# QuEraComputing/tsim

Hardware: AMD Instinct MI355X
Metric: detector shots/sec, 35-qubit distillation circuit, 1/2/4/8 MI355X (higher is better)
Workload: dtype int32

## Files before the change

tsim_amd/csrc/tsim_kernel_hw.hip.h:

```cpp
#pragma once
#include "tsim_kernels.hip.h"
#include "tsim_kernel4.hip.h"

namespace tsimk {

#define TSIMK_HW_MAX_CTX 8
struct HwMulti {
  int n_ctx, waves_per_list, max_lists;
  int comp_par;
  int par_words;
  uint32_t slot_cap;
  uint32_t hw_blocks;
  int comp4_off;
  uint32_t *feedback;
  SampleArgs ctx[TSIMK_HW_MAX_CTX];
};

__device__ __forceinline__ int hw_sum_i32(int v) {
#pragma unroll
  for (int o = 32; o > 0; o >>= 1) v += __shfl_xor(v, o, 64);
  return v;
}
__device__ __forceinline__ uint32_t hw_or_u32(uint32_t v) {
#pragma unroll
  for (int o = 32; o > 0; o >>= 1) v |= (uint32_t)__shfl_xor((int)v, o, 64);
  return v;
}

__device__ __forceinline__ uint32_t hw_bits(const uint32_t *par, uint32_t pos, uint32_t n) {
  const uint32_t w = pos >> 5, sh = pos & 31u;
  const uint32_t lo = par[w], hi = par[w + 1u];
  const uint32_t v = __builtin_amdgcn_alignbit(hi, lo, sh);
  return n >= 32u ? v : (v & ((1u << n) - 1u));
}

struct HwLevelOut {
  float re, im, re0, im0;
};

template <int W>
__device__ __forceinline__ void hw_phase1(const uint32_t *gimg, cptr lvl, const uint32_t (&x)[W], bool hasA, uint32_t flipA, bool hasB,
                                          uint32_t flipB, uint32_t *par, uint32_t pw, uint32_t wv, uint32_t nwv) {
  const uint32_t lane = threadIdx.x & 63u;
  const uint32_t n_rows = lvl[L_HWN];
  const uint32_t *rows = gimg + lvl[L_HWROWS];
  const uint32_t steps = (n_rows + 63u) >> 6;
  const uint32_t aw = flipA >> 5, as = flipA & 31u, bw = flipB >> 5, bs = flipB & 31u;
#pragma unroll 8
  for (uint32_t st = wv; st < steps; st += nwv) {
    const uint32_t r = st * 64u + lane;
    uint32_t pb = 0u, fa = 0u, fb = 0u;
    if (r < n_rows) {
      const uint32_t *q = rows + (size_t)r * (W + 1);
      uint32_t rw[W + 1];
#pragma unroll
      for (int w = 0; w <= W; ++w) rw[w] = q[w];
      uint32_t t = rw[W] & x[W - 1];
#pragma unroll
      for (int w = W - 2; w >= 0; --w) t = and_xor(rw[1 + w], x[w], t);
      pb = ((uint32_t)__builtin_popcount(t) + rw[0]) & 1u;
      uint32_t wa = rw[1], wb = rw[1];
#pragma unroll
      for (int w = 1; w < W; ++w) {
        wa = (aw == (uint32_t)w) ? rw[1 + w] : wa;
        wb = (bw == (uint32_t)w) ? rw[1 + w] : wb;
      }
      fa = (wa >> as) & 1u;
      fb = (wb >> bs) & 1u;
    }
    const unsigned long long m0 = __builtin_amdgcn_ballot_w64(pb != 0u);
    unsigned long long m1 = 0ull, m2 = 0ull, m3 = 0ull;
    if (hasA) m1 = __builtin_amdgcn_ballot_w64((pb ^ fa) != 0u);
    if (hasB) m2 = __builtin_amdgcn_ballot_w64((pb ^ fb) != 0u);
    if (hasA && hasB) m3 = __builtin_amdgcn_ballot_w64((pb ^ fa ^ fb) != 0u);
    if (lane == 0u) {
      par[2u * st] = (uint32_t)m0;
      par[2u * st + 1u] = (uint32_t)(m0 >> 32);
      if (hasA) { par[pw + 2u * st] = (uint32_t)m1; par[pw + 2u * st + 1u] = (uint32_t)(m1 >> 32); }
      if (hasB) { par[2u * pw + 2u * st] = (uint32_t)m2; par[2u * pw + 2u * st + 1u] = (uint32_t)(m2 >> 32); }
      if (hasA && hasB) { par[3u * pw + 2u * st] = (uint32_t)m3; par[3u * pw + 2u * st + 1u] = (uint32_t)(m3 >> 32); }
    }
  }
  if (lane == 0u && wv == (steps % nwv)) {
    par[2u * steps] = 0u;
    par[pw + 2u * steps] = 0u;
    par[2u * pw + 2u * steps] = 0u;
    par[3u * pw + 2u * steps] = 0u;
  }
}

typedef uint32_t hw_u32x4 __attribute__((ext_vector_type(4)));
struct HwRec {
  hw_u32x4 r0, r1, r2, r3;
};
__device__ __forceinline__ HwRec hw_load_rec(const uint32_t *gimg, cptr lvl, uint32_t g) {
  HwRec R;
  R.r0 = R.r1 = R.r2 = R.r3 = hw_u32x4{0u, 0u, 0u, 0u};
  if (g < lvl[L_G]) {
    const hw_u32x4 *q4 = reinterpret_cast<const hw_u32x4 *>(gimg + lvl[L_GRAPHS] + (size_t)g * G_WORDS);
    R.r0 = q4[0]; R.r1 = q4[1]; R.r2 = q4[2]; R.r3 = q4[3];
  }
  return R;
}

template <int W, bool DUAL>
__device__ __forceinline__ HwLevelOut hw_phase2(const uint32_t *gimg, cptr img, cptr lvl, const uint32_t *pa, const uint32_t *pa0, const HwRec &first) {
  const uint32_t G = lvl[L_G];
  const bool approx = (lvl[L_FLAGS] & TSIMK_LFLAG_APPROX) != 0;
  const bool fixed = (lvl[L_FLAGS] & TSIMK_LFLAG_FIXED) != 0;
  const uint32_t graphs = lvl[L_GRAPHS];
  const uint32_t lane = threadIdx.x & 63u;
  hw_u32x4 rec0 = first.r0, rec1 = first.r1, rec2 = first.r2, rec3 = first.r3;
  auto load_rec = [&](uint32_t g) {
    const hw_u32x4 *q4 = reinterpret_cast<const hw_u32x4 *>(gimg + graphs + (size_t)g * G_WORDS);
    rec0 = q4[0]; rec1 = q4[1]; rec2 = q4[2]; rec3 = q4[3];
  };
  LevelSum S, S0;
  for (uint32_t g0 = 0; g0 < G; g0 += 64u) {
    const uint32_t g = g0 + lane;
    const bool mine = g < G;
    int a = 0, b = 0, c = 0, d = 0, p = 0, a0 = 0, b0 = 0, c0 = 0, d0 = 0, p0 = 0;
    float tr = 0.0f, ti = 0.0f, tr0 = 0.0f, ti0 = 0.0f;
    if (mine && g0 > 0u) load_rec(g);
    if (mine) {
      const uint32_t n01 = rec0.x, n3h = rec0.y, flags = rec0.z, nD = rec0.w;
      const uint32_t start = rec2.x;
      static_assert(GF_N01 == 0 && GF_N3H == 1 && GF_FLAGS == 2 && GF_ND == 3 && GF_TBL == 5 && GF_N1 == 6 && GF_TBL2 == 7 && GF_HWROW == 8 &&
                        GF_APRE == 11 && GF_APIM == 12 && G_WORDS == 16, "record words are taken from the four 16-byte loads by position");
      GraphRec R;
      R.flags = flags; R.nD = nD; R.n1 = rec1.z; R.tbl = rec1.y; R.tbl2 = rec1.w;
      const uint32_t apre = rec2.w, apim = rec3.x;
      auto bits_of = [&](const uint32_t *pq) {
        GraphBits q;
        uint32_t pos = start;
        const uint32_t n0 = n01 & 0xFFFFu, n1 = n01 >> 16, n3 = n3h & 0xFFFFu;
        auto count = [&](uint32_t n) -> uint32_t {
          uint32_t m = (uint32_t)__builtin_popcount(hw_bits(pq, pos, n));
          for (uint32_t t0 = 32u; t0 < n; t0 += 32u) m += (uint32_t)__builtin_popcount(hw_bits(pq, pos + t0, n - t0));
          pos += n;
          return m;
        };
        q.m0 = count(n0);
        q.m1 = count(n1);
        q.m3 = count(n3);
        q.dbits = 0u;
        for (uint32_t t0 = 0; t0 < nD; t0 += 16u) {
          const uint32_t nt = min(16u, nD - t0);
          const uint32_t bits = hw_bits(pq, pos, 2u * nt);
          for (uint32_t t = 0; t < nt; ++t) q.dbits = (q.dbits << 2) | ((bits >> (2u * t)) & 3u);
          pos += 2u * nt;
        }
        q.lam = 0u;
        q.e = 0u;
        if (flags & TSIMK_GFLAG_LAM) { q.lam = hw_bits(pq, pos, 1u); pos += 1u; }
        if (flags & TSIMK_GFLAG_LIN) { q.e = hw_bits(pq, pos, 1u); pos += 1u; }
        const uint32_t nH = n3h >> 16;
        for (uint32_t t0 = 0; t0 < nH; t0 += 16u) {
          const uint32_t nt = min(16u, nH - t0);
          const uint32_t bits = hw_bits(pq, pos, 2u * nt);
          q.e ^= (uint32_t)__builtin_popcount(bits & (bits >> 1) & 0x55555555u);
          pos += 2u * nt;
        }
        return q;
      };
      const GraphBits q1 = bits_of(pa);
      graph_fast_value(gimg, R, fixed, q1, a, b, c, d, p);
      if (approx) level_term_approx(apre, apim, a, b, c, d, p, tr, ti);
      if constexpr (DUAL) {
        const GraphBits q0 = bits_of(pa0);
        graph_fast_value(gimg, R, fixed, q0, a0, b0, c0, d0, p0);
        if (approx) level_term_approx(apre, apim, a0, b0, c0, d0, p0, tr0, ti0);
      }
    }
    if (fixed) {
      S.sa += a; S.sb += b; S.sc += c; S.sd += d;
      if constexpr (DUAL) { S0.sa += a0; S0.sb += b0; S0.sc += c0; S0.sd += d0; }
    } else {
      const uint32_t n = min(64u, G - g0);
      for (uint32_t l = 0; l < n; ++l) {
        if (approx) {
          S.fre = __fadd_rn(S.fre, __uint_as_float((uint32_t)__builtin_amdgcn_readlane((int)__float_as_uint(tr), (int)l)));
          S.fim = __fadd_rn(S.fim, __uint_as_float((uint32_t)__builtin_amdgcn_readlane((int)__float_as_uint(ti), (int)l)));
          if constexpr (DUAL) {
            S0.fre = __fadd_rn(S0.fre, __uint_as_float((uint32_t)__builtin_amdgcn_readlane((int)__float_as_uint(tr0), (int)l)));
            S0.fim = __fadd_rn(S0.fim, __uint_as_float((uint32_t)__builtin_amdgcn_readlane((int)__float_as_uint(ti0), (int)l)));
          }
        } else {
          level_sum_exact(S, __builtin_amdgcn_readlane(a, (int)l), __builtin_amdgcn_readlane(b, (int)l), __builtin_amdgcn_readlane(c, (int)l),
                          __builtin_amdgcn_readlane(d, (int)l), __builtin_amdgcn_readlane(p, (int)l));
          if constexpr (DUAL)
            level_sum_exact(S0, __builtin_amdgcn_readlane(a0, (int)l), __builtin_amdgcn_readlane(b0, (int)l), __builtin_amdgcn_readlane(c0, (int)l),
                            __builtin_amdgcn_readlane(d0, (int)l), __builtin_amdgcn_readlane(p0, (int)l));
        }
      }
    }
  }
  if (fixed) {
    S.sa = hw_sum_i32(S.sa); S.sb = hw_sum_i32(S.sb); S.sc = hw_sum_i32(S.sc); S.sd = hw_sum_i32(S.sd);
    if constexpr (DUAL) { S0.sa = hw_sum_i32(S0.sa); S0.sb = hw_sum_i32(S0.sb); S0.sc = hw_sum_i32(S0.sc); S0.sd = hw_sum_i32(S0.sd); }
  }
  HwLevelOut o;
  o.re = o.im = o.re0 = o.im0 = 0.0f;
  level_finish(S, lvl, approx, fixed, o.re, o.im, nullptr);
  if constexpr (DUAL) level_finish(S0, lvl, approx, fixed, o.re0, o.im0, nullptr);
  return o;
}

template <int W, class FBit>
__device__ __forceinline__ void hw_component(const SampleArgs &A, cptr img, cptr comp, int ci, FBit fbit, unsigned long long shot, bool check,
                                             uint32_t *par, uint32_t pw, uint32_t (&out_w)[4]) {
  const uint32_t lane = threadIdx.x & 63u;
  const uint32_t wv = threadIdx.x >> 6, nwv = blockDim.x >> 6;
  const bool lead = wv == 0u;
  const uint32_t n_out = comp[C_NOUT], F = comp[C_F];
  cptr fsel = img + comp[C_FSEL];
  cptr levels = img + comp[C_LEVELS];
  cptr outpos = img + comp[C_OUTPOS];
  const uint32_t keybase = comp[C_KEYBASE];
  uint32_t *bit_word = par + 8u * pw;
  uint32_t x[W];
#pragma unroll
  for (int w2 = 0; w2 < W; w2 += 2) {
    const uint32_t j = 32u * (uint32_t)w2 + lane;
    const uint32_t raw = fbit(fsel[j < F ? j : 0u]);
    const unsigned long long m = __builtin_amdgcn_ballot_w64(j < F && raw != 0u);
    x[w2] = (uint32_t)m;
    if (w2 + 1 < W) x[w2 + 1] = (uint32_t)(m >> 32);
  }
  uint32_t u_bits = 0u;
  if (lead && n_out > 0u) {
    const uint32_t o = keybase + (lane < n_out ? lane : 0u);
    uint32_t x0 = (uint32_t)(shot >> 32), x1 = (uint32_t)shot;
    threefry2x32(subkey(A, o, 0), subkey(A, o, 1), x0, x1);
    u_bits = __float_as_uint(__uint_as_float(((x0 ^ x1) >> 9) | 0x3F800000u) - 1.0f);
  }
  auto set_bit = [&](uint32_t pos, bool on) {
    const uint32_t wi = pos >> 5, bm = 1u << (pos & 31u);
#pragma unroll
    for (int w = 0; w < W; ++w)
      if ((uint32_t)w == wi) x[w] = on ? (x[w] | bm) : (x[w] & ~bm);
  };
  HwRec cur = lead ? hw_load_rec(A.img, levels, lane) : HwRec{};
  hw_phase1<W>(A.img, levels, x, false, 0u, false, 0u, par, pw, wv, nwv);
  __syncthreads();
  float prev = 0.0f, maxdev = 0.0f;
  if (n_out > 0u) set_bit(F, true);
  if (lead) {
    const HwRec nxt = n_out > 0u ? hw_load_rec(A.img, levels + L_WORDS, lane) : HwRec{};
    const HwLevelOut n0 = hw_phase2<W, false>(A.img, img, levels, par, par, cur);
    prev = cabs32(n0.re, n0.im);
    cur = nxt;
  } else if (n_out > 0u) {
    hw_phase1<W>(A.img, levels + L_WORDS, x, false, 0u, check, F, par + 4u * pw, pw, wv - 1u, nwv - 1u);
  }
  __syncthreads();
  uint32_t prev_bit = 1u;
  for (uint32_t i = 0; i < n_out; ++i) {
    cptr lvl = levels + (i + 1) * L_WORDS;
    const uint32_t bitpos = F + i;
    uint32_t *buf = par + (((i + 1u) & 1u) ? 4u * pw : 0u);
    if (lead) {
      const uint32_t *pa = buf + (prev_bit ? 0u : pw);
      const HwRec nxt = i + 1u < n_out ? hw_load_rec(A.img, lvl + L_WORDS, lane) : HwRec{};
      float p1;
      if (check) {
        const HwLevelOut o = hw_phase2<W, true>(A.img, img, lvl, pa, pa + 2u * pw, cur);
        p1 = cabs32(o.re, o.im);
        const float p0 = cabs32(o.re0, o.im0);
        const float norm = __fdiv_rn(__fadd_rn(p0, p1), prev);
        maxdev = nanmax(maxdev, fabsf(__fsub_rn(norm, 1.0f)));
      } else {
        const HwLevelOut o = hw_phase2<W, false>(A.img, img, lvl, pa, pa, cur);
        p1 = cabs32(o.re, o.im);
      }
      const float u = __uint_as_float((uint32_t)__builtin_amdgcn_readlane((int)u_bits, (int)i));
      const bool bit = u < __fdiv_rn(p1, prev);
      prev = bit ? p1 : __fsub_rn(prev, p1);
      if (lane == 0u) *bit_word = bit ? 1u : 0u;
      cur = nxt;
    } else if (i + 1u < n_out) {
      uint32_t xn[W];
#pragma unroll
      for (int w = 0; w < W; ++w) xn[w] = x[w];
      const uint32_t np = bitpos + 1u, wi = np >> 5, bm = 1u << (np & 31u);
#pragma unroll
      for (int w = 0; w < W; ++w)
        if ((uint32_t)w == wi) xn[w] |= bm;
      hw_phase1<W>(A.img, lvl + L_WORDS, xn, true, bitpos, check, np, par + (((i + 2u) & 1u) ? 4u * pw : 0u), pw, wv - 1u, nwv - 1u);
    }
    __syncthreads();
    const bool bit = *bit_word != 0u;
    prev_bit = bit ? 1u : 0u;
    set_bit(bitpos, bit);
    if (i + 1u < n_out) set_bit(bitpos + 1u, true);
    const uint32_t dst = outpos[i];
    if (lane == 0u) {
#pragma unroll
      for (int w = 0; w < 4; ++w)
        if ((dst >> 5) == (uint32_t)w) out_w[w] |= (bit ? 1u : 0u) << (dst & 31u);
    }
  }
  if (check && A.norm_dev && threadIdx.x == 0u) A.norm_dev[ci] = maxdev;
  __syncthreads();
}


template <int WMAX>
__device__ __forceinline__ void hw_row(const SampleArgs &A, long long row, bool check, uint32_t *par, uint32_t pw, int only_comp) {
  cptr img = (cptr)(uintptr_t)A.img;
  const uint32_t lane = threadIdx.x & 63u;
  const unsigned long long shot = (unsigned long long)(A.shot_offset + row);
  const int WF32 = 2 * A.WF;
  const uint32_t *frow = reinterpret_cast<const uint32_t *>(A.f + row * A.WF);
  const uint32_t fw = (int)lane < WF32 ? frow[lane] : 0u;
  auto fbit = [&](uint32_t src) -> uint32_t {
    const uint32_t wv = (uint32_t)__shfl((int)fw, (int)(src >> 5), 64);
    return (wv >> (src & 31u)) & 1u;
  };
  uint32_t out_w[4] = {0u, 0u, 0u, 0u};
  if (only_comp < 0) {
    cptr dt = img + A.direct_off;
    for (int j0 = 0; j0 < A.n_direct; j0 += 64) {
      const int j = j0 + (int)lane;
      const bool mine = j < A.n_direct;
      const int jc = mine ? j : 0;
      const uint32_t s = dt[2 * jc], dst = mine ? dt[2 * jc + 1] : 0u;
      const uint32_t raw = fbit(s & 0x7FFFFFFFu);
      const uint32_t bit = mine ? (raw ^ (s >> 31)) : 0u;
#pragma unroll
      for (int w = 0; w < 4; ++w)
        if ((dst >> 5) == (uint32_t)w) out_w[w] |= bit << (dst & 31u);
    }
  }
  for (int ci = only_comp < 0 ? 0 : only_comp; ci < (only_comp < 0 ? A.n_comp : only_comp + 1); ++ci) {
    cptr comp = img + A.comp_off + ci * C_WORDS;
    switch (comp[C_W]) {
      case 1:
        hw_component<1>(A, img, comp, ci, fbit, shot, check, par, pw, out_w);
        break;
      case 2:
        if constexpr (WMAX >= 2) {
          hw_component<2>(A, img, comp, ci, fbit, shot, check, par, pw, out_w);
        }
        break;
      case 3:
      case 4:
        if constexpr (WMAX >= 4) {
          if (comp[C_W] == 3u) hw_component<3>(A, img, comp, ci, fbit, shot, check, par, pw, out_w);
          else hw_component<4>(A, img, comp, ci, fbit, shot, check, par, pw, out_w);
        }
        break;
      case 6:
      case 8:
        if constexpr (WMAX >= 8) {
          if (comp[C_W] == 6u) hw_component<6>(A, img, comp, ci, fbit, shot, check, par, pw, out_w);
          else hw_component<8>(A, img, comp, ci, fbit, shot, check, par, pw, out_w);
        }
        break;
      default: __builtin_trap();
    }
  }
#pragma unroll
  for (int w = 0; w < 4; ++w) out_w[w] = hw_or_u32(out_w[w]);
  if (threadIdx.x == 0u && only_comp >= 0) {
    if (A.out) {
      uint32_t *orow = reinterpret_cast<uint32_t *>(A.out + row * A.WO);
#pragma unroll
      for (int w = 0; w < 4; ++w)
        if (w < 2 * A.WO && out_w[w]) atomicOr(orow + w, out_w[w]);
    }
    if (A.out_compact) {
      const unsigned long long at = (unsigned long long)row * (unsigned long long)A.out_rb;
      uint32_t *base = reinterpret_cast<uint32_t *>(A.out_compact + (at & ~3ull));
      const uint32_t sh = 8u * (uint32_t)(at & 3ull);
#pragma unroll
      for (int w = 0; w < 5; ++w) {
        const uint32_t cur = w < 4 ? out_w[w < 4 ? w : 0] : 0u, below = w > 0 ? out_w[w > 0 ? w - 1 : 0] : 0u;
        const uint32_t v = sh ? ((cur << sh) | (below >> (32u - sh))) : cur;
        if (v) atomicOr(base + w, v);
      }
    }
  } else if (threadIdx.x == 0u) {
    if (A.out) {
      uint64_t *orow = A.out + row * A.WO;
      for (int w = 0; w < A.WO; ++w) orow[w] = (uint64_t)out_w[2 * w] | ((uint64_t)out_w[2 * w + 1] << 32);
    }
    if (A.out_compact) {
      uint8_t *dst = A.out_compact + row * A.out_rb;
      for (int k = 0; k < A.out_rb; ++k) dst[k] = (uint8_t)(out_w[k >> 2] >> (8 * (k & 3)));
    }
  }
}

template <int W, int NCH>
__global__ void __launch_bounds__(256) k_sample_hw(HwMulti M) {
  if constexpr (NCH > 0) {
    if (blockIdx.x >= M.hw_blocks) {
      over4_rows<4, NCH>(M.ctx, M.n_ctx, M.comp4_off, M.slot_cap, M.comp_par > 1, blockIdx.x - M.hw_blocks, gridDim.x - M.hw_blocks);
      return;
    }
  }
  __builtin_amdgcn_s_setprio(3);
  const uint32_t cp = (uint32_t)M.comp_par;
  const uint32_t wv = blockIdx.x / cp;
  const int only_comp = cp > 1u ? (int)(blockIdx.x - wv * cp) : -1;
  const uint32_t per_ctx = (uint32_t)(M.max_lists * M.waves_per_list);
  const uint32_t c = wv / per_ctx;
  if (c >= (uint32_t)M.n_ctx) return;
  const uint32_t r = wv - c * per_ctx;
  const SampleArgs &A = M.ctx[c];
  const uint32_t k = r / (uint32_t)M.waves_per_list, j = r - k * (uint32_t)M.waves_per_list;
  const uint32_t lane = threadIdx.x & 63u;
  if (M.feedback && blockIdx.x == 0u && threadIdx.x < 64u) {
    uint32_t cn = (int)lane < A.row_lists ? A.row_count[32u * lane] : 0u, mx = cn;
#pragma unroll
    for (int o = 32; o > 0; o >>= 1) {
      cn += (uint32_t)__shfl_xor((int)cn, o, 64);
      mx = max(mx, (uint32_t)__shfl_xor((int)mx, o, 64));
    }
    if (lane == 0u) {
      M.feedback[0] = cn;
      M.feedback[1] = mx;
      M.feedback[2] = (uint32_t)min(A.B, 0xFFFFFFFFll);
    }
  }
  if ((int)k >= A.row_lists) return;
  uint32_t n = A.row_count[32u * k];
  if (M.slot_cap) n = min(n, M.slot_cap);
  const uint32_t check_row = (A.no_check || !A.check_row) ? 0xFFFFFFFFu : *A.check_row;
  for (uint32_t slot = j; slot < n; slot += (uint32_t)M.waves_per_list) {
    const uint32_t entry = A.row_index[(size_t)k * A.row_list_cap + slot];
    if (only_comp >= 0) {
      if (!((entry >> (28 + only_comp)) & 1u)) continue;
      const uint32_t row = entry & 0x0FFFFFFFu;
      hw_row<W>(A, (long long)row, row == check_row, tsimk_lds, (uint32_t)M.par_words, only_comp);
    } else {
      hw_row<W>(A, (long long)entry, entry == check_row, tsimk_lds, (uint32_t)M.par_words, -1);
    }
  }
}

}
```

tsim_amd/csrc/tsim_sample.hip:

```cpp
#include "tsim_internal.hip.h"

#include <chrono>
#include "tsim_kernel4h.hip.h"
#include "tsim_filter.hip.h"
#include "tsim_lw_pass.hip.h"
#include "tsim_lw_multi.hip.h"
#include "tsim_lw_fast.hip.h"
#include "tsim_kernel4w.hip.h"
#include "tsim_kernel_hw.hip.h"
#include "tsim_direct.hip.h"
#include "tsim_lw_fastm.hip.h"
#include "tsim_sample_internal.hip.h"
#include "tsim_noise_fused.hip.h"

using namespace tsimk;
using namespace tsimhost;

thread_local TsimNoiseRequest *g_noise_req = nullptr;
HostMarks *g_marks = nullptr;


int prof_event(tsim_program *p, hipStream_t s, int tag) {
  if (p->ev_used == p->ev_pool.size()) {
    hipEvent_t e;
// ... 165 lines not shown
    }
    pl.defer = pipelined && pl.use_tables && !dense && !pl.need_overflow && pl.hard_kernel && p->knobs.defer &&
               p->v4 && !(p->profiling && !p->prof_light);
  }
  return pl;
}

static int slots_now_ready(tsim_program *p) {
  p->slots_ready = true;
  return 0;
}
static thread_local const LaunchPlan *g_carry_plan = nullptr;

void hard_geometry(tsim_program *p, int WF, int WO) {
  constexpr int NW = TSIM_HARD_NW;
  const size_t tile_b = (size_t)p->v4_max_nch * 16 * p->v4_gt * 16;
  const size_t fixed_b = (size_t)(2 * WF + 2 * WO) * 64 * 4 + (size_t)NW * 8 * 64 * 4;
  const size_t budget = (size_t)kHardLdsKb * 1024;
  p->h_group_tiles = fixed_b + tile_b <= budget ? (int)std::min<size_t>(TSIMK_H_MAX_GROUP_TILES, (budget - fixed_b) / tile_b) : 0;
  p->h_lds = fixed_b + (size_t)std::max(1, p->h_group_tiles) * tile_b;
}

static bool hw_eligible(tsim_program *p, const SampleArgs &a, int n_ctx) {
  int wmax = 1;
  for (int w : p->comp_w) wmax = std::max(wmax, w);
  const uint32_t fb_rows = p->h_feedback ? p->h_feedback[0] : 0u;
  return p->fast && p->knobs.hard_wave && wmax <= 4 && a.WF <= 32 && a.WO <= 2 && p->hw_max_rows < 60000 &&
         (unsigned long long)fb_rows * (unsigned)n_ctx <= (unsigned long long)p->knobs.hard_wave_rows;
}
static int launch_over(tsim_program *p, const SampleArgs *ctx, int n_ctx, uint32_t slot_begin, bool masked, hipStream_t hs, bool fill_chip = false) {
  Over4Multi M{};
  M.n_ctx = n_ctx;
  M.comp4_off = p->comp4_off;
  M.slot_begin = slot_begin;
  M.masked = masked ? 1 : 0;
  for (int i = 0; i < n_ctx; ++i) {
    M.ctx[i] = ctx[i];
    M.ctx[i].kernarg_off = (int)(offsetof(Over4Multi, ctx) + (size_t)i * sizeof(SampleArgs));
    M.ctx[i].row_slot_begin = 0;
    M.ctx[i].row_slot_end = 0;
  }
  const int blk = 256;
  const size_t tile_bytes = std::max((size_t)p->v4_max_nch * 16, (size_t)p->v4_max_sent) * p->v4_gt * 16;
  const size_t lds4 = (size_t)(2 * ctx[0].WF + 2 * ctx[0].WO) * blk * 4 + 2 * tile_bytes;
  if (lds4 > (p->v4_max_nch == 32 ? 160 : 64) * 1024) return tsim_fail(TSIM_ENOTSUP, "v4 kernel needs %zu B of LDS", lds4);
  const unsigned grid = (unsigned)p->n_cu * (fill_chip ? (unsigned)std::max<size_t>(1, std::min<size_t>(2048 / blk, (160 * 1024) / (lds4 + 256))) : 1u);
  ++p->path_count[TP_OVER];
  switch (p->v4_max_nch) {
#define TSIM_LO(N) case N: hipLaunchKernelGGL((k_sample4_over<4, N>), dim3(grid), dim3(blk), lds4, hs, M); break;
    TSIM_LO(2) TSIM_LO(4) TSIM_LO(6) TSIM_LO(8) TSIM_LO(10) TSIM_LO(12) TSIM_LO(14) TSIM_LO(20)
#undef TSIM_LO
    case 32: {
      auto kfn = k_sample4_over<4, 32>;
      if (!(p->x4_attr_set & 1u)) { HIP_TRY(hipFuncSetAttribute((const void *)kfn, hipFuncAttributeMaxDynamicSharedMemorySize, 160 * 1024 - 4096)); p->x4_attr_set |= 1u; }
      hipLaunchKernelGGL(kfn, dim3(grid), dim3(blk), lds4, hs, M);
    } break;
    default: hipLaunchKernelGGL((k_sample4_over<4, 16>), dim3(grid), dim3(blk), lds4, hs, M); break;
  }
  HIP_TRY(hipGetLastError());
  return 0;
}
static bool over_available(const tsim_program *p) { return p->v4 && p->knobs.hard_overflow; }

static int launch_hw(tsim_program *p, const SampleArgs *ctx, int n_ctx, int max_lists, hipStream_t hs, bool partial, bool with_feedback = true) {
  int wmax = 1;
  for (int w : p->comp_w) wmax = std::max(wmax, w);
  const uint32_t fb_max = p->h_feedback ? p->h_feedback[1] : 192u;
  HwMulti H{};
  H.n_ctx = n_ctx;
  H.max_lists = max_lists;
  H.waves_per_list = (int)std::max(8u, std::min(128u, std::min(fb_max, 4096u) * 2u + 8u));
  H.feedback = with_feedback ? p->d_feedback : nullptr;
  for (int i = 0; i < n_ctx; ++i) {
    H.ctx[i] = ctx[i];
    H.ctx[i].kernarg_off = (int)(offsetof(HwMulti, ctx) + (size_t)i * sizeof(SampleArgs));
  }
  H.comp_par = partial ? (int)p->comps.size() : 1;
  const bool workers = over_available(p);
  H.slot_cap = workers ? (uint32_t)H.waves_per_list * 4u : 0u;
  H.comp4_off = p->comp4_off;
  const unsigned gridw = (unsigned)((long long)H.n_ctx * H.max_lists * H.waves_per_list * H.comp_par);
  H.hw_blocks = gridw;
  H.par_words = (int)(2 * ((p->hw_max_rows + 63) / 64) + 2);
  size_t ldsw = (size_t)H.par_words * 8 * 4 + 16;
  unsigned grid = gridw;
  if (workers) {
    const size_t tile_bytes = std::max((size_t)p->v4_max_nch * 16, (size_t)p->v4_max_sent) * p->v4_gt * 16;
    ldsw = std::max(ldsw, (size_t)(2 * ctx[0].WF + 2 * ctx[0].WO) * 256 * 4 + 2 * tile_bytes);
    if (ldsw > (p->v4_max_nch == 32 ? 160 : 64) * 1024) return tsim_fail(TSIM_ENOTSUP, "v4 kernel needs %zu B of LDS", ldsw);
    grid += (unsigned)(2 * p->n_cu);
  }
  const int nch = workers ? p->v4_max_nch : 0;
  ++p->path_count[TP_HW];
#define TSIM_LHW(WV, N) case N: hipLaunchKernelGGL((k_sample_hw<WV, N>), dim3(grid), dim3(256), ldsw, hs, H); break;
  if (wmax == 1) switch (nch) {
    TSIM_LHW(1, 0) TSIM_LHW(1, 2) TSIM_LHW(1, 4) TSIM_LHW(1, 6) TSIM_LHW(1, 8) TSIM_LHW(1, 10) TSIM_LHW(1, 12) TSIM_LHW(1, 14) TSIM_LHW(1, 16)
    default: return tsim_fail(TSIM_ESTATE, "bad chunk count %d", nch);
  } else if (wmax > 4) {
    if (nch != 0 || wmax > 8) return tsim_fail(TSIM_ESTATE, "block-per-row kernel: %d parameter words, %d chunks", wmax, nch);
    hipLaunchKernelGGL((k_sample_hw<8, 0>), dim3(grid), dim3(256), ldsw, hs, H);
  } else if (wmax > 2) {
    switch (nch) {
      TSIM_LHW(4, 0) TSIM_LHW(4, 20)
      case 32: {
        auto kfn = k_sample_hw<4, 32>;
        if (!(p->x4_attr_set & 2u)) { HIP_TRY(hipFuncSetAttribute((const void *)kfn, hipFuncAttributeMaxDynamicSharedMemorySize, 160 * 1024 - 4096)); p->x4_attr_set |= 2u; }
        hipLaunchKernelGGL(kfn, dim3(grid), dim3(256), ldsw, hs, H);
      } break;
      default: return tsim_fail(TSIM_ESTATE, "hard-row workers need chunk tables (%d chunks)", nch);
    }
  } else switch (nch) {
    TSIM_LHW(2, 0) TSIM_LHW(2, 2) TSIM_LHW(2, 4) TSIM_LHW(2, 6) TSIM_LHW(2, 8) TSIM_LHW(2, 10) TSIM_LHW(2, 12) TSIM_LHW(2, 14) TSIM_LHW(2, 16)
    default: return tsim_fail(TSIM_ESTATE, "bad chunk count %d", nch);
  }
#undef TSIM_LHW
  HIP_TRY(hipGetLastError());
  return 0;
}

int flush_batch(tsim_program *p) {
  if (p->deferred.empty()) {
    p->flush_inline = nullptr;
    return 0;
  }
  constexpr int NW = TSIM_HARD_NW;
  const unsigned long long seq = p->batch_next++;
  int bl = 0;
  hipStream_t hs = p->slots[3].side;
  if (p->flush_inline) {
    hs = p->flush_inline;
    bl = 2;
    for (int k = 0; k < 4; ++k)
      if (hs == p->slots[1 + k].side) bl = 2 + k;
    p->flush_inline = nullptr;
    p->inline_seen = true;
  }
  Hard4Multi M{};
  M.n_ctx = (int)p->deferred.size();
  const uint32_t fb_max = p->h_feedback ? p->h_feedback[1] : 192u;
  const uint32_t fb_sum0 = p->h_feedback ? p->h_feedback[0] : 0xFFFFFFFFu;
  const bool many0 = over_available(p) && fb_sum0 != 0xFFFFFFFFu && (unsigned long long)fb_sum0 * (unsigned)p->deferred.size() > 16384ull;
  const int hb = many0 ? 1 : (int)std::max(1u, std::min(4u, (std::min(fb_max, 192u) + 32u + 63u) / 64u));
  int max_lists = 1;
  for (int sidx : p->deferred) max_lists = std::max(max_lists, p->slots[sidx].ctx.row_lists);
  M.blocks_per_ctx = hb * max_lists + 1;
  M.group_tiles = p->h_group_tiles;
  M.loop_stride = hb * 64;
  M.comp4_off = p->comp4_off;
  M.feedback = p->d_feedback;
  bool lane_used[2] = {false, false};
  for (int i = 0; i < M.n_ctx; ++i) {
    tsim_program::Slot &d = p->slots[p->deferred[i]];
    for (int k = 0; k < 2; ++k)
      if (d.p1_stream == p->slots[1 + k].side) lane_used[k] = true;
    M.ctx[i] = d.ctx;
    M.ctx[i].kernarg_off = (int)(offsetof(Hard4Multi, ctx) + (size_t)i * sizeof(SampleArgs));
    if (d.ctx_check) M.check_mask |= 1 << i;
  }
  for (int k = 0; k < 2; ++k)
    if (lane_used[k] && p->slots[1 + k].side != hs) {
      if (!p->lane_ev[k]) HIP_TRY(hipEventCreateWithFlags(&p->lane_ev[k], hipEventDisableTiming));
      HIP_TRY(hipEventRecord(p->lane_ev[k], p->slots[1 + k].side));
      HIP_TRY(hipStreamWaitEvent(hs, p->lane_ev[k], 0));
    }
  const bool partial = p->slots[p->deferred[0]].partial;
  if (partial || hw_eligible(p, M.ctx[0], M.n_ctx) || !p->v4) {
    if (int r = launch_hw(p, M.ctx, M.n_ctx, max_lists, hs, partial)) return r;
// ... 1122 lines not shown
  if (!d_row_index || !d_row_count) return tsim_fail(TSIM_EINVAL, "row list is NULL");
  if (B >= (1ll << 32)) return tsim_fail(TSIM_ENOTSUP, "row indices are 32-bit");
  hipStream_t s = stream ? (hipStream_t)stream : p->stream;
  return launch_sample(p, d_f, B, num_f, key_hi, key_lo, shot_offset, d_out, d_max_norm_dev, s, d_row_index,
                       d_row_count);
}

extern "C" int tsim_postselect_device(tsim_program *p, const uint64_t *d_f, int64_t B, int32_t num_f,
                                      const uint64_t *d_mask, const uint64_t *d_ref, uint64_t *d_out,
                                      uint32_t *d_row_index, uint32_t *d_row_count, uint8_t *d_discarded,
                                      void *stream) {
  if (int r = tsim_need_final(p)) return r;
  if (int r = tsim_set_device(p)) return r;
  if (B < 0 || num_f < 0) return tsim_fail(TSIM_EINVAL, "negative size");
  if (B >= (1ll << 32)) return tsim_fail(TSIM_ENOTSUP, "row indices are 32-bit");
  if (p->max_f_index >= num_f) return tsim_fail(TSIM_EINVAL, "program references f index %d but num_f=%d", p->max_f_index, num_f);
  if (!d_mask || !d_out || !d_row_index || !d_row_count) return tsim_fail(TSIM_EINVAL, "NULL buffer");
  hipStream_t s = stream ? (hipStream_t)stream : p->stream;
  HIP_TRY(hipMemsetAsync(d_row_count, 0, 4, s));
  if (B == 0 || p->num_outputs == 0) return TSIM_OK;
  FilterArgs a;
  a.img = p->d_img;
  a.f = d_f;
  a.out = d_out;
  a.mask = d_mask;
  a.ref = d_ref;
  a.row_index = d_row_index;
  a.row_count = d_row_count;
  a.discarded = d_discarded;
  a.B = B;
  a.WF = num_f == 0 ? 0 : std::max(1, (num_f + 63) / 64);
  a.WO = (p->num_outputs + 63) / 64;
  a.n_direct = p->n_direct;
  a.direct_off = p->direct_off;
  int block = 256;
  size_t lds = (size_t)(2 * a.WF + 2 * a.WO) * block * 4;
  if (lds > 60 * 1024) { block = 64; lds = (size_t)(2 * a.WF + 2 * a.WO) * block * 4; }
  if (lds > 60 * 1024) return tsim_fail(TSIM_ENOTSUP, "num_f + num_outputs too large for LDS staging (%zu B)", lds);
  hipLaunchKernelGGL(k_direct_filter, dim3((unsigned)((B + block - 1) / block)), dim3(block), lds, s, a);
  HIP_TRY(hipGetLastError());
  return TSIM_OK;
}
extern "C" int tsim_sample_batch(tsim_program *p, const uint8_t *f, int64_t B, int32_t num_f, uint32_t key_hi,
                                 uint32_t key_lo, int64_t shot_offset, uint8_t *out, int32_t out_packed,
                                 float *max_norm_dev) {
  if (int r = tsim_need_final(p)) return r;
  if (int r = tsim_set_device(p)) return r;
  if (B < 0 || num_f < 0) return tsim_fail(TSIM_EINVAL, "negative B/num_f");
  if (B == 0 || p->num_outputs == 0) return 0;
  if (!out) return tsim_fail(TSIM_EINVAL, "out is NULL");
  if (!f && num_f > 0) return tsim_fail(TSIM_EINVAL, "f is NULL");
  const int WF = std::max(1, (num_f + 63) / 64), WO = (p->num_outputs + 63) / 64;
  hipStream_t s = p->stream;
  if (int r = tsim_ensure_scratch(p, 0, (size_t)B * std::max(1, num_f))) return r;
  if (int r = tsim_ensure_scratch(p, 1, (size_t)B * WF * 8)) return r;
  if (int r = tsim_ensure_scratch(p, 2, (size_t)B * WO * 8)) return r;
  if (num_f > 0) {
    HIP_TRY(hipMemcpyAsync(p->scratch[0], f, (size_t)B * num_f, hipMemcpyHostToDevice, s));
    if (int r = tsim_launch_pack(p, (const uint8_t *)p->scratch[0], B, num_f, (uint64_t *)p->scratch[1], s)) return r;
  }
  if (int r = launch_sample(p, (const uint64_t *)p->scratch[1], B, num_f, key_hi, key_lo, shot_offset,
                            (uint64_t *)p->scratch[2], p->d_dev, s))
    return r;
  if (out_packed) {
    HIP_TRY(hipMemcpyAsync(out, p->scratch[2], (size_t)B * WO * 8, hipMemcpyDeviceToHost, s));
  } else {
    if (int r = tsim_ensure_scratch(p, 3, (size_t)B * p->num_outputs)) return r;
    if (int r = tsim_launch_unpack(p, (const uint64_t *)p->scratch[2], B, p->num_outputs, (uint8_t *)p->scratch[3], s)) return r;
    HIP_TRY(hipMemcpyAsync(out, p->scratch[3], (size_t)B * p->num_outputs, hipMemcpyDeviceToHost, s));
  }
  if (max_norm_dev && shot_offset == 0 && !p->comps.empty())
    HIP_TRY(hipMemcpyAsync(max_norm_dev, p->d_dev, p->comps.size() * 4, hipMemcpyDeviceToHost, s));
  HIP_TRY(hipStreamSynchronize(s));
  return TSIM_OK;
}
#ifdef TSIMK_LW_TRACE
extern "C" int tsim_debug_lw_trace(unsigned long long *out) {
  HIP_TRY(hipDeviceSynchronize());
  HIP_TRY(hipMemcpyFromSymbol(out, HIP_SYMBOL(tsimk::tsimk_lw_trace), 16 * 32 * 8));
  return 0;
}
#endif

#ifdef TSIMK_WIDE_TRACE
extern "C" int tsim_debug_wide_trace(unsigned long long *out) {
  HIP_TRY(hipDeviceSynchronize());
  HIP_TRY(hipMemcpyFromSymbol(out, HIP_SYMBOL(tsimk::tsimk_wide_trace), 24 * 8));
  unsigned long long z[24] = {};
  HIP_TRY(hipMemcpyToSymbol(HIP_SYMBOL(tsimk::tsimk_wide_trace), z, 24 * 8));
  return 0;
}
#endif

extern "C" int tsim_profile_enable(tsim_program *p, int32_t on) {
  if (int r = tsim_need_final(p)) return r;
  if (int r = tsim_set_device(p)) return r;
  if (!on && p->ev_used) { if (int r = prof_drain(p)) return r; }
  p->profiling = on != 0;
  p->prof_light = on == 2;
  p->prof_counter = 0;
  return TSIM_OK;
}

extern "C" int tsim_profile_set_sampling(tsim_program *p, int32_t every) {
  if (!p || every < 1) return tsim_fail(TSIM_EINVAL, "bad argument");
  p->prof_every = every;
  p->prof_counter = 0;
  return TSIM_OK;
}

extern "C" int tsim_profile_read(tsim_program *p, double *kernel_ms, int64_t *launches, int32_t reset) {
  if (int r = tsim_need_final(p)) return r;
  if (int r = tsim_set_device(p)) return r;
  if (int r = prof_drain(p)) return r;
  if (kernel_ms) *kernel_ms = p->prof_ms;
  if (launches) *launches = p->prof_launches;
  if (reset) {
    p->prof_ms = 0.0;
    p->prof_launches = 0;
    for (double &v : p->prof_stage_ms) v = 0.0;
  }
  return TSIM_OK;
}

extern "C" int tsim_profile_read_steps(tsim_program *p, int64_t *steps, int32_t reset) {
  if (int r = tsim_need_final(p)) return r;
  if (!steps) return tsim_fail(TSIM_EINVAL, "NULL argument");
  *steps = p->prof_steps;
  if (reset) p->prof_steps = 0;
  return TSIM_OK;
}

extern "C" int tsim_profile_read_stages(tsim_program *p, double stage_ms[3]) {
  if (int r = tsim_need_final(p)) return r;
  if (int r = tsim_set_device(p)) return r;
  if (!stage_ms) return tsim_fail(TSIM_EINVAL, "NULL argument");
  if (int r = prof_drain(p)) return r;
  stage_ms[0] = p->prof_stage_ms[PROF_PASS1];
  stage_ms[1] = p->prof_stage_ms[PROF_HARD];
  stage_ms[2] = p->prof_stage_ms[PROF_FULL];
  return TSIM_OK;
}
```

Baseline: 78.32 billion.

## Split dual check evaluation across waves and triple-buffer row parities

The lead wave used to evaluate both the p1 and the p0 (norm-check) amplitudes serially in a DUAL phase2. Now a second (and third) wave computes the p0 and initial-level values in parallel, passing results through a small LDS exchange area. Parity buffers go from two to three so phase1 for level i+2 can overlap phase2 of earlier levels, and the first outcome level is peeled out of the loop. LDS use per block grows, fewer waves are left for the row pass, and optional timestamp instrumentation is added behind a compile flag.

```diff
diff --git a/tsim_amd/csrc/tsim_kernel_hw.hip.h b/tsim_amd/csrc/tsim_kernel_hw.hip.h
--- a/tsim_amd/csrc/tsim_kernel_hw.hip.h
+++ b/tsim_amd/csrc/tsim_kernel_hw.hip.h
@@ -35,7 +35,7 @@
 }
 
 struct HwLevelOut {
-  float re, im, re0, im0;
+  float re, im;
 };
 
 template <int W>
@@ -103,8 +103,34 @@
   return R;
 }
 
-template <int W, bool DUAL>
-__device__ __forceinline__ HwLevelOut hw_phase2(const uint32_t *gimg, cptr img, cptr lvl, const uint32_t *pa, const uint32_t *pa0, const HwRec &first) {
+#ifndef TSIMK_HW_STAMPS
+#define TSIMK_HW_STAMPS 0
+#endif
+#define TSIMK_HW_STAMP_EVENTS 128
+#define TSIMK_HW_STAMP_WORDS (8 * 4 * TSIMK_HW_STAMP_EVENTS)
+enum { HWS_BEGIN = 0, HWS_BITS = 1, HWS_GATHER = 2, HWS_SUM = 3, HWS_FINISH = 4, HWS_BARRIER = 5, HWS_ROWPASS = 6 };
+#if TSIMK_HW_STAMPS
+__device__ unsigned long long tsimk_hw_stamps[TSIMK_HW_STAMP_WORDS];
+__shared__ uint32_t tsimk_hw_stamp_row;
+__shared__ uint32_t tsimk_hw_stamp_base;
+__device__ __forceinline__ void hw_stamp(uint32_t link, uint32_t phase) {
+  const uint32_t ev = 8u * link + phase, base = tsimk_hw_stamp_base;
+  if (base != 0xFFFFFFFFu && (threadIdx.x & 63u) == 0u && ev < TSIMK_HW_STAMP_EVENTS)
+    tsimk_hw_stamps[base + (threadIdx.x >> 6) * TSIMK_HW_STAMP_EVENTS + ev] = (unsigned long long)wall_clock64();
+}
+__device__ __forceinline__ void hw_stamp_component(int ci) {
+  __syncthreads();
+  if (threadIdx.x == 0u)
+    tsimk_hw_stamp_base = tsimk_hw_stamp_row == 0xFFFFFFFFu ? 0xFFFFFFFFu : (tsimk_hw_stamp_row * 4u + (uint32_t)min(ci, 3)) * 4u * TSIMK_HW_STAMP_EVENTS;
+  __syncthreads();
+}
+#else
+__device__ __forceinline__ void hw_stamp(uint32_t, uint32_t) {}
+__device__ __forceinline__ void hw_stamp_component(int) {}
+#endif
+
+template <int W>
+__device__ __forceinline__ HwLevelOut hw_phase2(const uint32_t *gimg, cptr lvl, const uint32_t *pa, const HwRec &first, uint32_t step) {
   const uint32_t G = lvl[L_G];
   const bool approx = (lvl[L_FLAGS] & TSIMK_LFLAG_APPROX) != 0;
   const bool fixed = (lvl[L_FLAGS] & TSIMK_LFLAG_FIXED) != 0;
@@ -115,12 +141,13 @@
     const hw_u32x4 *q4 = reinterpret_cast<const hw_u32x4 *>(gimg + graphs + (size_t)g * G_WORDS);
     rec0 = q4[0]; rec1 = q4[1]; rec2 = q4[2]; rec3 = q4[3];
   };
-  LevelSum S, S0;
+  hw_stamp(step, HWS_BEGIN);
+  LevelSum S;
   for (uint32_t g0 = 0; g0 < G; g0 += 64u) {
     const uint32_t g = g0 + lane;
     const bool mine = g < G;
-    int a = 0, b = 0, c = 0, d = 0, p = 0, a0 = 0, b0 = 0, c0 = 0, d0 = 0, p0 = 0;
-    float tr = 0.0f, ti = 0.0f, tr0 = 0.0f, ti0 = 0.0f;
+    int a = 0, b = 0, c = 0, d = 0, p = 0;
+    float tr = 0.0f, ti = 0.0f;
     if (mine && g0 > 0u) load_rec(g);
     if (mine) {
       const uint32_t n01 = rec0.x, n3h = rec0.y, flags = rec0.z, nD = rec0.w;
@@ -130,81 +157,74 @@
       GraphRec R;
       R.flags = flags; R.nD = nD; R.n1 = rec1.z; R.tbl = rec1.y; R.tbl2 = rec1.w;
       const uint32_t apre = rec2.w, apim = rec3.x;
-      auto bits_of = [&](const uint32_t *pq) {
-        GraphBits q;
-        uint32_t pos = start;
-        const uint32_t n0 = n01 & 0xFFFFu, n1 = n01 >> 16, n3 = n3h & 0xFFFFu;
-        auto count = [&](uint32_t n) -> uint32_t {
-          uint32_t m = (uint32_t)__builtin_popcount(hw_bits(pq, pos, n));
-          for (uint32_t t0 = 32u; t0 < n; t0 += 32u) m += (uint32_t)__builtin_popcount(hw_bits(pq, pos + t0, n - t0));
-          pos += n;
-          return m;
-        };
-        q.m0 = count(n0);
-        q.m1 = count(n1);
-        q.m3 = count(n3);
-        q.dbits = 0u;
-        for (uint32_t t0 = 0; t0 < nD; t0 += 16u) {
-          const uint32_t nt = min(16u, nD - t0);
-          const uint32_t bits = hw_bits(pq, pos, 2u * nt);
-          for (uint32_t t = 0; t < nt; ++t) q.dbits = (q.dbits << 2) | ((bits >> (2u * t)) & 3u);
-          pos += 2u * nt;
-        }
-        q.lam = 0u;
-        q.e = 0u;
-        if (flags & TSIMK_GFLAG_LAM) { q.lam = hw_bits(pq, pos, 1u); pos += 1u; }
-        if (flags & TSIMK_GFLAG_LIN) { q.e = hw_bits(pq, pos, 1u); pos += 1u; }
-        const uint32_t nH = n3h >> 16;
-        for (uint32_t t0 = 0; t0 < nH; t0 += 16u) {
-          const uint32_t nt = min(16u, nH - t0);
-          const uint32_t bits = hw_bits(pq, pos, 2u * nt);
-          q.e ^= (uint32_t)__builtin_popcount(bits & (bits >> 1) & 0x55555555u);
-          pos += 2u * nt;
-        }
-        return q;
+      GraphBits q;
+      uint32_t pos = start;
+      const uint32_t n0 = n01 & 0xFFFFu, n1 = n01 >> 16, n3 = n3h & 0xFFFFu;
+      auto count = [&](uint32_t n) -> uint32_t {
+        uint32_t m = (uint32_t)__builtin_popcount(hw_bits(pa, pos, n));
+        for (uint32_t t0 = 32u; t0 < n; t0 += 32u) m += (uint32_t)__builtin_popcount(hw_bits(pa, pos + t0, n - t0));
+        pos += n;
+        return m;
       };
-      const GraphBits q1 = bits_of(pa);
-      graph_fast_value(gimg, R, fixed, q1, a, b, c, d, p);
+      q.m0 = count(n0);
+      q.m1 = count(n1);
+      q.m3 = count(n3);
+      q.dbits = 0u;
+      for (uint32_t t0 = 0; t0 < nD; t0 += 16u) {
+        const uint32_t nt = min(16u, nD - t0);
+        const uint32_t bits = hw_bits(pa, pos, 2u * nt);
+        for (uint32_t t = 0; t < nt; ++t) q.dbits = (q.dbits << 2) | ((bits >> (2u * t)) & 3u);
+        pos += 2u * nt;
+      }
+      q.lam = 0u;
+      q.e = 0u;
+      if (flags & TSIMK_GFLAG_LAM) { q.lam = hw_bits(pa, pos, 1u); pos += 1u; }
+      if (flags & TSIMK_GFLAG_LIN) { q.e = hw_bits(pa, pos, 1u); pos += 1u; }
+      const uint32_t nH = n3h >> 16;
+      for (uint32_t t0 = 0; t0 < nH; t0 += 16u) {
+        const uint32_t nt = min(16u, nH - t0);
+        const uint32_t bits = hw_bits(pa, pos, 2u * nt);
+        q.e ^= (uint32_t)__builtin_popcount(bits & (bits >> 1) & 0x55555555u);
+        pos += 2u * nt;
+      }
+#if TSIMK_HW_STAMPS
+      asm volatile("s_waitcnt lgkmcnt(0)" ::: "memory");
+      hw_stamp(step, HWS_BITS);
+#endif
+      graph_fast_value(gimg, R, fixed, q, a, b, c, d, p);
+#if TSIMK_HW_STAMPS
+      asm volatile("s_waitcnt vmcnt(0)" ::: "memory");
+      hw_stamp(step, HWS_GATHER);
+#endif
       if (approx) level_term_approx(apre, apim, a, b, c, d, p, tr, ti);
-      if constexpr (DUAL) {
-        const GraphBits q0 = bits_of(pa0);
-        graph_fast_value(gimg, R, fixed, q0, a0, b0, c0, d0, p0);
-        if (approx) level_term_approx(apre, apim, a0, b0, c0, d0, p0, tr0, ti0);
-      }
     }
     if (fixed) {
       S.sa += a; S.sb += b; S.sc += c; S.sd += d;
-      if constexpr (DUAL) { S0.sa += a0; S0.sb += b0; S0.sc += c0; S0.sd += d0; }
     } else {
       const uint32_t n = min(64u, G - g0);
       for (uint32_t l = 0; l < n; ++l) {
         if (approx) {
           S.fre = __fadd_rn(S.fre, __uint_as_float((uint32_t)__builtin_amdgcn_readlane((int)__float_as_uint(tr), (int)l)));
           S.fim = __fadd_rn(S.fim, __uint_as_float((uint32_t)__builtin_amdgcn_readlane((int)__float_as_uint(ti), (int)l)));
-          if constexpr (DUAL) {
-            S0.fre = __fadd_rn(S0.fre, __uint_as_float((uint32_t)__builtin_amdgcn_readlane((int)__float_as_uint(tr0), (int)l)));
-            S0.fim = __fadd_rn(S0.fim, __uint_as_float((uint32_t)__builtin_amdgcn_readlane((int)__float_as_uint(ti0), (int)l)));
-          }
         } else {
           level_sum_exact(S, __builtin_amdgcn_readlane(a, (int)l), __builtin_amdgcn_readlane(b, (int)l), __builtin_amdgcn_readlane(c, (int)l),
                           __builtin_amdgcn_readlane(d, (int)l), __builtin_amdgcn_readlane(p, (int)l));
-          if constexpr (DUAL)
-            level_sum_exact(S0, __builtin_amdgcn_readlane(a0, (int)l), __builtin_amdgcn_readlane(b0, (int)l), __builtin_amdgcn_readlane(c0, (int)l),
-                            __builtin_amdgcn_readlane(d0, (int)l), __builtin_amdgcn_readlane(p0, (int)l));
         }
       }
     }
   }
   if (fixed) {
     S.sa = hw_sum_i32(S.sa); S.sb = hw_sum_i32(S.sb); S.sc = hw_sum_i32(S.sc); S.sd = hw_sum_i32(S.sd);
-    if constexpr (DUAL) { S0.sa = hw_sum_i32(S0.sa); S0.sb = hw_sum_i32(S0.sb); S0.sc = hw_sum_i32(S0.sc); S0.sd = hw_sum_i32(S0.sd); }
-  }
+  }
+  hw_stamp(step, HWS_SUM);
   HwLevelOut o;
-  o.re = o.im = o.re0 = o.im0 = 0.0f;
+  o.re = o.im = 0.0f;
   level_finish(S, lvl, approx, fixed, o.re, o.im, nullptr);
-  if constexpr (DUAL) level_finish(S0, lvl, approx, fixed, o.re0, o.im0, nullptr);
   return o;
 }
+
+#define TSIMK_HW_BUFS 3
+enum { HWX_BIT = 0 , HWX_P0 = 2 , HWX_PREV0 = 4, HWX_P1 = 5, HWX_U0 = 6, HWX_WORDS = 8 };
 
 template <int W, class FBit>
 __device__ __forceinline__ void hw_component(const SampleArgs &A, cptr img, cptr comp, int ci, FBit fbit, unsigned long long shot, bool check,
@@ -217,7 +237,9 @@
   cptr levels = img + comp[C_LEVELS];
   cptr outpos = img + comp[C_OUTPOS];
   const uint32_t keybase = comp[C_KEYBASE];
-  uint32_t *bit_word = par + 8u * pw;
+  hw_stamp_component(ci);
+  uint32_t *xw = par + (uint32_t)(4 * TSIMK_HW_BUFS) * pw;
+  auto buf_of = [&](uint32_t level) { return par + (level % (uint32_t)TSIMK_HW_BUFS) * 4u * pw; };
   uint32_t x[W];
 #pragma unroll
   for (int w2 = 0; w2 < W; w2 += 2) {
@@ -233,6 +255,7 @@
     uint32_t x0 = (uint32_t)(shot >> 32), x1 = (uint32_t)shot;
     threefry2x32(subkey(A, o, 0), subkey(A, o, 1), x0, x1);
     u_bits = __float_as_uint(__uint_as_float(((x0 ^ x1) >> 9) | 0x3F800000u) - 1.0f);
+    if (lane == 0u) xw[HWX_U0] = u_bits;
   }
   auto set_bit = [&](uint32_t pos, bool on) {
     const uint32_t wi = pos >> 5, bm = 1u << (pos & 31u);
@@ -240,44 +263,89 @@
     for (int w = 0; w < W; ++w)
       if ((uint32_t)w == wi) x[w] = on ? (x[w] | bm) : (x[w] & ~bm);
   };
-  HwRec cur = lead ? hw_load_rec(A.img, levels, lane) : HwRec{};
+  float prev = 0.0f, maxdev = 0.0f;
+  if (n_out == 0u) {
+    const HwRec cur = lead ? hw_load_rec(A.img, levels, lane) : HwRec{};
+    hw_phase1<W>(A.img, levels, x, false, 0u, false, 0u, par, pw, wv, nwv);
+    __syncthreads();
+    if (lead) {
+      const HwLevelOut n0 = hw_phase2<W>(A.img, levels, par, cur, 0u);
+      prev = cabs32(n0.re, n0.im);
+    }
+    if (check && A.norm_dev && threadIdx.x == 0u) A.norm_dev[ci] = maxdev;
+    __syncthreads();
+    return;
+  }
+  const uint32_t nev = check ? 3u : 2u;
+  HwRec cur = wv < nev ? hw_load_rec(A.img, levels + (lead ? 0u : L_WORDS), lane) : HwRec{};
   hw_phase1<W>(A.img, levels, x, false, 0u, false, 0u, par, pw, wv, nwv);
+  set_bit(F, true);
+  hw_phase1<W>(A.img, levels + L_WORDS, x, false, 0u, check, F, buf_of(1u), pw, wv, nwv);
+  hw_stamp(0u, HWS_ROWPASS);
   __syncthreads();
-  float prev = 0.0f, maxdev = 0.0f;
-  if (n_out > 0u) set_bit(F, true);
-  if (lead) {
-    const HwRec nxt = n_out > 0u ? hw_load_rec(A.img, levels + L_WORDS, lane) : HwRec{};
-    const HwLevelOut n0 = hw_phase2<W, false>(A.img, img, levels, par, par, cur);
-    prev = cabs32(n0.re, n0.im);
+  hw_stamp(0u, HWS_BARRIER);
+  if (wv < nev) {
+    const HwRec nxt = (n_out > 1u && wv < nev - 1u) ? hw_load_rec(A.img, levels + 2u * L_WORDS, lane) : HwRec{};
+    const HwLevelOut o = hw_phase2<W>(A.img, levels + (lead ? 0u : L_WORDS), lead ? par : buf_of(1u) + (wv == 2u ? 2u * pw : 0u), cur, 1u);
+    const float v = cabs32(o.re, o.im);
+    if (lane == 0u) xw[lead ? HWX_PREV0 : (wv == 1u ? HWX_P1 : HWX_P0)] = __float_as_uint(v);
     cur = nxt;
-  } else if (n_out > 0u) {
-    hw_phase1<W>(A.img, levels + L_WORDS, x, false, 0u, check, F, par + 4u * pw, pw, wv - 1u, nwv - 1u);
+    hw_stamp(1u, HWS_FINISH);
+  } else if (n_out > 1u) {
+    uint32_t xn[W];
+#pragma unroll
+    for (int w = 0; w < W; ++w) xn[w] = x[w];
+    const uint32_t np = F + 1u, wi = np >> 5, bm = 1u << (np & 31u);
+#pragma unroll
+    for (int w = 0; w < W; ++w)
+      if ((uint32_t)w == wi) xn[w] |= bm;
+    hw_phase1<W>(A.img, levels + 2u * L_WORDS, xn, true, F, check, np, buf_of(2u), pw, wv - nev, nwv - nev);
+    hw_stamp(1u, HWS_ROWPASS);
   }
   __syncthreads();
-  uint32_t prev_bit = 1u;
-  for (uint32_t i = 0; i < n_out; ++i) {
+  hw_stamp(1u, HWS_BARRIER);
+  uint32_t prev_bit;
+  float chk_p1 = 0.0f, chk_prev = 0.0f;
+  {
+    const float prev0 = __uint_as_float(xw[HWX_PREV0]), p1 = __uint_as_float(xw[HWX_P1]), u = __uint_as_float(xw[HWX_U0]);
+    const bool bit = u < __fdiv_rn(p1, prev0);
+    if (lead) {
+      if (check) {
+        const float p0 = __uint_as_float(xw[HWX_P0]);
+        const float norm = __fdiv_rn(__fadd_rn(p0, p1), prev0);
+        maxdev = nanmax(maxdev, fabsf(__fsub_rn(norm, 1.0f)));
+      }
+      prev = bit ? p1 : __fsub_rn(prev0, p1);
+    }
+    prev_bit = bit ? 1u : 0u;
+    set_bit(F, bit);
+    if (n_out > 1u) set_bit(F + 1u, true);
+    const uint32_t dst = outpos[0];
+    const uint32_t ov = (lane == 0u && bit) ? 1u << (dst & 31u) : 0u;
+#pragma unroll
+    for (int w = 0; w < 4; ++w) out_w[w] |= (dst >> 5) == (uint32_t)w ? ov : 0u;
+  }
+  const uint32_t nb = check ? 2u : 1u;
+  for (uint32_t i = 1; i < n_out; ++i) {
     cptr lvl = levels + (i + 1) * L_WORDS;
     const uint32_t bitpos = F + i;
-    uint32_t *buf = par + (((i + 1u) & 1u) ? 4u * pw : 0u);
-    if (lead) {
-      const uint32_t *pa = buf + (prev_bit ? 0u : pw);
+    if (wv < nb) {
+      const uint32_t *pa = buf_of(i + 1u) + (prev_bit ? 0u : pw) + (lead ? 0u : 2u * pw);
       const HwRec nxt = i + 1u < n_out ? hw_load_rec(A.img, lvl + L_WORDS, lane) : HwRec{};
-      float p1;
-      if (check) {
-        const HwLevelOut o = hw_phase2<W, true>(A.img, img, lvl, pa, pa + 2u * pw, cur);
-        p1 = cabs32(o.re, o.im);
-        const float p0 = cabs32(o.re0, o.im0);
-        const float norm = __fdiv_rn(__fadd_rn(p0, p1), prev);
-        maxdev = nanmax(maxdev, fabsf(__fsub_rn(norm, 1.0f)));
-      } else {
-        const HwLevelOut o = hw_phase2<W, false>(A.img, img, lvl, pa, pa, cur);
-        p1 = cabs32(o.re, o.im);
-      }
-      const float u = __uint_as_float((uint32_t)__builtin_amdgcn_readlane((int)u_bits, (int)i));
-      const bool bit = u < __fdiv_rn(p1, prev);
-      prev = bit ? p1 : __fsub_rn(prev, p1);
-      if (lane == 0u) *bit_word = bit ? 1u : 0u;
+      const HwLevelOut o = hw_phase2<W>(A.img, lvl, pa, cur, i + 1u);
+      const float pv = cabs32(o.re, o.im);
+      if (lead) {
+        const float u = __uint_as_float((uint32_t)__builtin_amdgcn_readlane((int)u_bits, (int)i));
+        const bool bit = u < __fdiv_rn(pv, prev);
+        chk_p1 = pv;
+        chk_prev = prev;
+        prev = bit ? pv : __fsub_rn(prev, pv);
+        if (lane == 0u) xw[HWX_BIT + (i & 1u)] = bit ? 1u : 0u;
+      } else if (lane == 0u) {
+        xw[HWX_P0 + (i & 1u)] = __float_as_uint(pv);
+      }
       cur = nxt;
+      hw_stamp(i + 1u, HWS_FINISH);
     } else if (i + 1u < n_out) {
       uint32_t xn[W];
 #pragma unroll
@@ -286,19 +354,24 @@
 #pragma unroll
       for (int w = 0; w < W; ++w)
         if ((uint32_t)w == wi) xn[w] |= bm;
-      hw_phase1<W>(A.img, lvl + L_WORDS, xn, true, bitpos, check, np, par + (((i + 2u) & 1u) ? 4u * pw : 0u), pw, wv - 1u, nwv - 1u);
+      hw_phase1<W>(A.img, lvl + L_WORDS, xn, true, bitpos, check, np, buf_of(i + 2u), pw, wv - nb, nwv - nb);
+      hw_stamp(i + 1u, HWS_ROWPASS);
     }
     __syncthreads();
-    const bool bit = *bit_word != 0u;
+    hw_stamp(i + 1u, HWS_BARRIER);
+    const bool bit = xw[HWX_BIT + (i & 1u)] != 0u;
+    if (lead && check) {
+      const float p0 = __uint_as_float(xw[HWX_P0 + (i & 1u)]);
+      const float norm = __fdiv_rn(__fadd_rn(p0, chk_p1), chk_prev);
+      maxdev = nanmax(maxdev, fabsf(__fsub_rn(norm, 1.0f)));
+    }
     prev_bit = bit ? 1u : 0u;
     set_bit(bitpos, bit);
     if (i + 1u < n_out) set_bit(bitpos + 1u, true);
     const uint32_t dst = outpos[i];
-    if (lane == 0u) {
-#pragma unroll
-      for (int w = 0; w < 4; ++w)
-        if ((dst >> 5) == (uint32_t)w) out_w[w] |= (bit ? 1u : 0u) << (dst & 31u);
-    }
+    const uint32_t ov = (lane == 0u && bit) ? 1u << (dst & 31u) : 0u;
+#pragma unroll
+    for (int w = 0; w < 4; ++w) out_w[w] |= (dst >> 5) == (uint32_t)w ? ov : 0u;
   }
   if (check && A.norm_dev && threadIdx.x == 0u) A.norm_dev[ci] = maxdev;
   __syncthreads();
@@ -430,6 +503,13 @@
   const uint32_t check_row = (A.no_check || !A.check_row) ? 0xFFFFFFFFu : *A.check_row;
   for (uint32_t slot = j; slot < n; slot += (uint32_t)M.waves_per_list) {
     const uint32_t entry = A.row_index[(size_t)k * A.row_list_cap + slot];
+#if TSIMK_HW_STAMPS
+    __syncthreads();
+    if (threadIdx.x == 0u) {
+      const uint32_t row_of = only_comp >= 0 ? (entry & 0x0FFFFFFFu) : entry;
+      tsimk_hw_stamp_row = row_of == check_row ? 1u : (blockIdx.x < cp ? 0u : 0xFFFFFFFFu);
+    }
+#endif
     if (only_comp >= 0) {
       if (!((entry >> (28 + only_comp)) & 1u)) continue;
       const uint32_t row = entry & 0x0FFFFFFFu;
diff --git a/tsim_amd/csrc/tsim_sample.hip b/tsim_amd/csrc/tsim_sample.hip
--- a/tsim_amd/csrc/tsim_sample.hip
+++ b/tsim_amd/csrc/tsim_sample.hip
@@ -271,7 +271,7 @@
   const unsigned gridw = (unsigned)((long long)H.n_ctx * H.max_lists * H.waves_per_list * H.comp_par);
   H.hw_blocks = gridw;
   H.par_words = (int)(2 * ((p->hw_max_rows + 63) / 64) + 2);
-  size_t ldsw = (size_t)H.par_words * 8 * 4 + 16;
+  size_t ldsw = ((size_t)H.par_words * 4 * TSIMK_HW_BUFS + tsimk::HWX_WORDS) * 4;
   unsigned grid = gridw;
   if (workers) {
     const size_t tile_bytes = std::max((size_t)p->v4_max_nch * 16, (size_t)p->v4_max_sent) * p->v4_gt * 16;
@@ -1560,6 +1560,16 @@
 }
 #endif
 
+#if TSIMK_HW_STAMPS
+extern "C" int tsim_debug_hw_stamps(unsigned long long *out) {
+  HIP_TRY(hipDeviceSynchronize());
+  HIP_TRY(hipMemcpyFromSymbol(out, HIP_SYMBOL(tsimk::tsimk_hw_stamps), TSIMK_HW_STAMP_WORDS * 8));
+  static unsigned long long z[TSIMK_HW_STAMP_WORDS] = {};
+  HIP_TRY(hipMemcpyToSymbol(HIP_SYMBOL(tsimk::tsimk_hw_stamps), z, sizeof(z)));
+  return 0;
+}
+#endif
+
 #ifdef TSIMK_WIDE_TRACE
 extern "C" int tsim_debug_wide_trace(unsigned long long *out) {
   HIP_TRY(hipDeviceSynchronize());
```

After: 78.63 billion (median of 2 runs). About the same (+0.4%).
